# Totoro97/f2-nerf

Hardware: AMD Instinct MI355X
Metric: training ray-samples/s (ngp_fox) (higher is better)
Workload: dtype f16; 1 GPU; ngp_fox wanjinyou.yaml, 8192 rays/batch/GPU, 2^19 x16 table, the first 2188 iterations of training from the fresh-initialised table (fineness 8.7), synthetic random-pose rays, full train step (fwd+bwd+Adam+octree update); rays_per_batch=8192, parallelism=ray-dp1

## Files before the change

### f2-nerf_amd/capi.py

```python
import ctypes
import os

import torch

from . import build

_lib = None
ABI_VERSION = 13


class F2nError(RuntimeError):
    pass


def lib():
    global _lib
    if _lib is None:
        if not os.path.exists(build.LIB):
            raise F2nError("native library %s is missing: run `python -c 'import __graft_entry__ as g; g.build()'` "
                           "(there is no CPU fallback)" % build.LIB)
        _lib = ctypes.CDLL(build.LIB)
        _lib.f2n_build_info.restype = ctypes.c_char_p
        if _lib.f2n_abi_version() != ABI_VERSION:
            raise F2nError("%s reports ABI version %d, this binding is written for %d: rebuild (__graft_entry__.build())"
# ... 454 lines not shown


def draw_ray_batch(n_rays, u01, image_set, height, width, poses, intri, dist_params, images, cam_bounds, cam_indices, ij, rays_o,
                   rays_d, gt_colors, bounds):
    _ck(lib().f2n_draw_ray_batch(_stream(), _i(n_rays), _p(u01, "f32"), _p(image_set, "i32"), _i(int(image_set.numel())), _i(height),
                                 _i(width), _p(poses, "f32"), _p(intri, "f32"), _p(dist_params, "f32"), _p(images, "f32", True),
                                 _p(cam_bounds, "f32"), _p(cam_indices, "i32"), _p(ij, "i32"), _p(rays_o, "f32"), _p(rays_d, "f32"),
                                 _p(gt_colors, "f32", True), _p(bounds, "f32")), "f2n_draw_ray_batch")


def gather_pixels(n, height, width, images, cam_bounds, cam_idx, ij, gt_colors, bounds):
    _ck(lib().f2n_gather_pixels(_stream(), _i(n), _i(height), _i(width), _p(images, "f32", True), _p(cam_bounds, "f32", True),
                                _p(cam_idx, "i32"), _p(ij, "i32"), _p(gt_colors, "f32", True), _p(bounds, "f32", True)),
        "f2n_gather_pixels")


def early_stop(n_rays, pts_se, f0, f0_stride, dt, weights, alphas, mask, kept):
    _ck(lib().f2n_early_stop(_stream(), _i(n_rays), _p(pts_se, "i32"), _p(f0, "f32"), _i(f0_stride), _p(dt, "f32"),
                             _p(weights, "f32"), _p(alphas, "f32"), _p(mask, "i32"), _p(kept, "i32")), "f2n_early_stop")


def compact_samples(n_rays, old_se, new_se, mask, pts, dirs, dt, t, anchors, o_pts, o_dirs, o_dt, o_t, o_anchors):
    _ck(lib().f2n_compact_samples(_stream(), _i(n_rays), _p(old_se, "i32"), _p(new_se, "i32"), _p(mask, "i32"),
                                  _p(pts, "f32"), _p(dirs, "f32"), _p(dt, "f32"), _p(t, "f32"), _p(anchors, "i32"),
                                  _p(o_pts, "f32"), _p(o_dirs, "f32"), _p(o_dt, "f32"), _p(o_t, "f32"),
                                  _p(o_anchors, "i32")), "f2n_compact_samples")


def compact_samples_src(n_rays, old_se, new_se, mask, pts, dirs, dt, t, anchors, o_pts, o_dirs, o_dt, o_t, o_anchors, o_src,
                        o_vol=None, ray_val=None, o_ray_val=None):
    _ck(lib().f2n_compact_samples_src(_stream(), _i(n_rays), _p(old_se, "i32"), _p(new_se, "i32"), _p(mask, "i32"),
                                      _p(pts, "f32"), _p(dirs, "f32"), _p(dt, "f32"), _p(t, "f32"), _p(anchors, "i32"),
                                      _p(o_pts, "f32"), _p(o_dirs, "f32"), _p(o_dt, "f32"), _p(o_t, "f32"),
                                      _p(o_anchors, "i32"), _p(o_src, "i32"), _p(o_vol, "i32", True), _p(ray_val, "i32", True),
                                      _p(o_ray_val, "i32", True)), "f2n_compact_samples_src")


def oct_visible_cams(n_boxes, n_cams, boxes, c2w, bounds, fx, fy, cx, cy, res_h, res_w, pix_i, pix_j, visible):
    _ck(lib().f2n_oct_visible_cams(_stream(), _i(n_boxes), _i(n_cams), _p(boxes, "f32"), _p(c2w, "f32"), _p(bounds, "f32"), _f(fx),
                                   _f(fy), _f(cx), _f(cy), _i(res_h), _i(res_w), _p(pix_i, "f32"), _p(pix_j, "f32"),
                                   _p(visible, "u8")), "f2n_oct_visible_cams")


def march_noise(n, u, fineness, out):
    _ck(lib().f2n_march_noise(_stream(), _i(n), _p(u, "f32"), _f(fineness), _p(out, "f32")), "f2n_march_noise")


def composite_fwd(n_rays, pts_se, feat, dt, t, rgb, bg, colors, disparity, depth, weights, f0_stride=16, out_vars=None):
    _ck(lib().f2n_composite_fwd(_stream(), _i(n_rays), _p(pts_se, "i32"), _p(feat, "f32"), _i(f0_stride), _p(dt, "f32"),
                                _p(t, "f32"), _p(rgb, "f32"), _p(bg, "f32"), _p(colors, "f32"), _p(disparity, "f32"),
                                _p(depth, "f32"), _p(weights, "f32"), _p(out_vars, "f32", True)), "f2n_composite_fwd")


def composite_bwd(n_rays, pts_se, feat, dt, t, rgb, bg, dcolors, ddisp, ddepth, dweights, gs_progress, drgb, dfeat, f0_stride=16,
                  df0_stride=16, var_weights=None, dvars=None):
    _ck(lib().f2n_composite_bwd(_stream(), _i(n_rays), _p(pts_se, "i32"), _p(feat, "f32"), _i(f0_stride), _p(dt, "f32"),
                                _p(t, "f32"), _p(rgb, "f32"), _p(bg, "f32"), _p(dcolors, "f32", True), _p(ddisp, "f32", True),
                                _p(ddepth, "f32", True), _p(dweights, "f32", True), _f(gs_progress), _p(drgb, "f32"),
                                _p(dfeat, "f32"), _i(df0_stride), _p(var_weights, "f32", True), _p(dvars, "f32", True)),
        "f2n_composite_bwd")


def weight_var_fwd(n_rays, weights, pts_se, out):
    _ck(lib().f2n_weight_var_fwd(_stream(), _i(n_rays), _p(weights, "f32"), _p(pts_se, "i32"), _p(out, "f32")),
        "f2n_weight_var_fwd")


# ... 808 lines not shown
```

### f2-nerf_amd/csrc/host/Renderer.cpp

```cpp
#include "Renderer.h"

#include <hip/hip_runtime_api.h>

#include <cstdio>
#include <cstdlib>
#include <mutex>

namespace f2n {

using torch::autograd::AutogradContext;
using torch::autograd::variable_list;

namespace {

struct CompositeFunction : public torch::autograd::Function<CompositeFunction> {
  static variable_list forward(AutogradContext* ctx, Tensor feat, Tensor rgb, Tensor dt, Tensor t, Tensor bg, Tensor se,
                               double gs_progress) {
    ctx->set_materialize_grads(false);
    const int n_rays = se.size(0), m = feat.size(0);
    Tensor colors = torch::empty({n_rays, 3}, DevF32()), disparity = torch::empty({n_rays}, DevF32());
    Tensor depth = torch::empty({n_rays}, DevF32()), weights = torch::empty({m}, DevF32());
    F2N_TIMED_CALL("composite_fwd", f2n_composite_fwd(CurStream(), n_rays, I32P(se), F32P(feat), F2N_MLP_OUT_PAD, F32P(dt), F32P(t), F32P(rgb), F32P(bg),
                               F32P(colors), F32P(disparity), F32P(depth), F32P(weights), nullptr));
    ctx->save_for_backward({feat, rgb, dt, t, bg, se});
// ... 116 lines not shown
  return float(dp_count_host_.data_ptr<int32_t>()[0]) / (float(n_rays) * float(dp_world_));
}

void Renderer::ResolvePendingCount() {
  if (!count_pending_) return;
  count_pending_ = false;
  {
    F2N_HOST_SCOPE("wait.kept");
    kept_wait_ev_->synchronize();
  }
  const int n_kept = n_kept_words_.Read(1);
  last_n_kept_pts_ = n_kept;
  total_kept_pts_ += n_kept;
  DigestKept(pending_count_seq_, n_kept);
  auto* gdp = global_data_pool_;
  if (dp_world_ > 1) {
    if (dp_sum_mirrored_) {
      const float per_ray = float(n_kept_words_.Read(0)) / (float(dp_sum_rays_) * float(dp_world_));
      gdp->meaningful_sampled_pts_per_ray_ = gdp->meaningful_sampled_pts_per_ray_ * 0.9f + per_ray * 0.1f;
      RecordEma(pending_count_seq_ - 1);
    }
    dp_sum_mirrored_ = false;
    return;
  }
  gdp->meaningful_sampled_pts_per_ray_ = gdp->meaningful_sampled_pts_per_ray_ * 0.9f + KeptPerRayForEma(n_kept, pending_count_rays_) * 0.1f;
  RecordEma(pending_count_seq_);
}

RenderFront Renderer::SampleAndFilter(const Tensor& rays_o, const Tensor& rays_d, const Tensor& bounds, const Tensor& emb_idx,
                                      bool async_count) {
  F2N_HOST_SCOPE("step.sample_and_filter");
  auto* gdp = global_data_pool_;
  ResolvePendingCount();
  if (gdp->mode_ == RunningMode::TRAIN) DebugSkew(2);
  auto* field = static_cast<Hash3DAnchored*>(scene_field_.get());
  const bool train = gdp->mode_ == RunningMode::TRAIN;
  const int n_rays = rays_o.size(0);
  spec_start_recorded_ = false;
  spec_start_is_consumed_ = false;
  if (train && async_count && (next_batch_.valid || next2_batch_.valid) && speculative_sampling_ != 0) {
    if (rays_off_main_ && side_shared_ && side_shared_->seq > 0) spec_start_is_consumed_ = true;
    else spec_start_ev_.record();
    spec_start_recorded_ = true;
  }
  auto* ps = static_cast<PersSampler*>(pts_sampler_.get());
  if (train) {
    KeepOnlyPending(rays_o, rays_d, next_batch_.valid ? next_batch_.rays_o : Tensor(), next_batch_.valid ? next_batch_.rays_d : Tensor(),
                    next2_batch_.valid ? next2_batch_.rays_o : Tensor(), next2_batch_.valid ? next2_batch_.rays_d : Tensor());
    const int slot = FindPending(rays_o, rays_d);
    if (slot >= 0) PreSampleFinish(slot);
  } else {
    DropPendingSamples();
  }
  bool wait_for_pack = false;
  int pack_slot = 0;
  auto pack_done = [&]() {
    if (wait_for_pack) presample_done_ev_[pack_slot].block(c10::hip::getCurrentHIPStreamMasqueradingAsCUDA());
    wait_for_pack = false;
  };
  if (train && PresampleMatches(rays_o, rays_d)) {
    sample_result_ = std::move(presampled_);
    if (presample_async_) {
      wait_for_pack = true;
      pack_slot = presample_slot_;
      consumed_side_samples_ = true;
    }
// ... 136 lines not shown
      }
      pack_done();
      if (digest_taps_ && train) {
        DigestTap(TAP_PTS_PRE, sample_result_.pts);
        DigestTap(TAP_DT_PRE, sample_result_.dt);
        DigestTap(TAP_ANCHORS_PRE, sample_result_.anchors.select(1, 0));
      }
      f0_full = field->QueryDensityPreAct(pts_full, anchors_full, true, keep_prepass_outputs_,
                                          keep_prepass_outputs_ && prepass_planes_cache_);
      f0p = F32P(f0_full) + front;
      if (digest_taps_ && train) DigestTap(TAP_EDGE, pts_full.narrow(0, 0, front));
      fr.edge_cache_row = 0;
      fr.sample_cache_row = front;
    } else {
      pack_done();
      if (digest_taps_ && train) {
        DigestTap(TAP_PTS_PRE, sample_result_.pts);
        DigestTap(TAP_DT_PRE, sample_result_.dt);
        DigestTap(TAP_ANCHORS_PRE, sample_result_.anchors.select(1, 0));
      }
      f0_full = field->QueryDensityPreAct(sample_result_.pts, sample_result_.anchors, true, keep_prepass_outputs_,
                                          keep_prepass_outputs_ && prepass_planes_cache_);
      f0p = F32P(f0_full);
    }
    if (digest_taps_ && train) {
      DigestTap(TAP_PTS, sample_result_.pts);
      DigestTap(TAP_DT, sample_result_.dt);
      DigestTap(TAP_ANCHORS, sample_result_.anchors.select(1, 0));
      DigestTap(TAP_F0, f0_full);
      DigestTap(TAP_BG, bg_color);
    }
    Tensor weights = torch::empty({n_all_pts}, DevF32()), alphas = torch::empty({n_all_pts}, DevF32());
    Tensor mask = torch::empty({n_all_pts}, DevI32()), kept = torch::empty({n_rays}, DevI32());
    if (train) ps->EarlyStopAndVote(sample_result_, f0p, weights, alphas, mask, kept);
    else F2N_TIMED_CALL("early_stop", f2n_early_stop(st, n_rays, I32P(sample_result_.pts_idx_bounds), f0p, 1, F32P(sample_result_.dt),
                            F32P(weights), F32P(alphas), I32P(mask), I32P(kept)));
    const bool octree_first = train && async_count;
    auto octree_update_issued = [&]() {
      octree_ready_ev_.record();
      const int nslot = next_batch_.valid ? FindPending(next_batch_.rays_o, next_batch_.rays_d) : -1;
      if (nslot >= 0 && pend_[nslot].s.speculative && !pend_[nslot].s.completed && PreSampleSpecComplete(nslot)) after_octree_update_ = nullptr;
      else if (nslot >= 0 && pend_[nslot].s.completed) after_octree_update_ = nullptr;
      if (after_octree_update_) {
        auto f = std::move(after_octree_update_);
        after_octree_update_ = nullptr;
        f();
      }
    };
    Tensor new_se = torch::empty({n_rays, 2}, DevI32()), total = torch::empty({1}, DevI32());
    n_kept_words_.Ensure(2);
    bool scan_issued = false;
    if (octree_first) {
      PersSampler::ScanArgs sa;
      sa.n = n_rays; sa.counts = I32P(kept); sa.start_end = I32P(new_se); sa.total = I32P(total);
      if (train && dp_world_ > 1 && dp_count_.defined()) {
        sa.mirror = n_kept_words_.Dev(0); sa.also = I32P(dp_count_); sa.n_also = 1;
        dp_sum_mirrored_ = true;
        dp_sum_rays_ = dp_count_rays_;
      } else {
        sa.mirror = n_kept_words_.Dev(1);
      }
      ps->FinishOctUpdate(&sa);
      scan_issued = true;
      octree_update_issued();
    }
    const bool dp_lagged = train && dp_world_ > 1 && octree_first;
    if (scan_issued) {
    } else if (dp_lagged && dp_count_.defined()) {
      F2N_CALL(f2n_segment_scan_ex(st, n_rays, I32P(kept), I32P(new_se), I32P(total), n_kept_words_.Dev(0), I32P(dp_count_), 1));
      dp_sum_mirrored_ = true;
      dp_sum_rays_ = dp_count_rays_;
    } else {
      F2N_CALL(f2n_segment_scan_ex(st, n_rays, I32P(kept), I32P(new_se), I32P(total), n_kept_words_.Dev(1), nullptr, 0));
    }
    kept_wait_ev_ = scan_issued ? &octree_ready_ev_ : &n_kept_ev_;
    if (!scan_issued) n_kept_ev_.record();
    if (digest_taps_ && train) DigestTap(TAP_SURVIVORS, new_se);
    if (dp_lagged) {
      dp_count_ = total;
      dp_count_rays_ = n_rays;
    } else if (train && dp_world_ > 1) {
      dp_count_ = total.clone();
    }
    if (train && !octree_first) ps->FinishOctUpdate();
    if (train && dp_world_ > 1 && !dp_lagged) {
      if (!dp_count_host_.defined()) dp_count_host_ = torch::empty({1}, torch::TensorOptions().dtype(torch::kInt32).pinned_memory(true));
      dp_count_host_.copy_(dp_count_, true);
      dp_count_ev_.record();
    }
    if (train && !octree_first) octree_update_issued();
    if (async_count) {
      n_kept = n_all_pts;
      if (train) {
        count_pending_ = true;
        pending_count_rays_ = n_rays;
        pending_count_seq_ = cur_seq_;
      }
      fr.dyn = true;
      fr.n_kept_dev = total;
    } else {
      kept_wait_ev_->synchronize();
      n_kept = n_kept_words_.Read(1);
      if (train && after_count_readback_) after_count_readback_();
      last_n_kept_pts_ = n_kept;
      if (train) total_kept_pts_ += n_kept;
    }
    const int64_t so = fr.dyn ? 2 * (int64_t) n_edge : 0;
    const int64_t eo = fr.dyn ? 0 : n_kept;
    if (!edges_cached) {
      pts_all = torch::empty({n_kept + 2 * n_edge, 3}, DevF32());
      vol_all = torch::empty({n_kept + 2 * n_edge}, DevI32());
    }
    es.pts = pts_all.slice(0, so, so + n_kept);
    es.dirs = torch::empty({n_kept, 3}, DevF32());
    es.dt = torch::empty({n_kept}, DevF32());
    es.t = torch::empty({n_kept}, DevF32());
    es.anchors = torch::empty({n_kept, 3}, DevI32());
    es.first_oct_dis = sample_result_.first_oct_dis;
    es.pts_idx_bounds = new_se;
    src_rows = torch::empty({std::max(n_kept, 1)}, DevI32());
    const bool want_emb = train && use_app_emb_ && emb_idx.defined();
    Tensor emb_contig;
    if (want_emb) {
      emb_contig = emb_idx.contiguous();
      CheckDev(emb_contig, torch::kInt32, "emb_idx");
      fr.sample_emb_idx = torch::empty({std::max(n_kept, 1)}, DevI32());
    }
    F2N_TIMED_CALL("compact_samples", f2n_compact_samples_src(st, n_rays, I32P(sample_result_.pts_idx_bounds), I32P(new_se), I32P(mask),
                                 F32P(sample_result_.pts), F32P(sample_result_.dirs), F32P(sample_result_.dt),
                                 F32P(sample_result_.t), I32P(sample_result_.anchors), F32P(pts_all) + 3 * so, F32P(es.dirs),
                                 F32P(es.dt), F32P(es.t), I32P(es.anchors), I32P(src_rows), I32P(vol_all) + so,
                                 want_emb ? I32P(emb_contig) : nullptr, want_emb ? I32P(fr.sample_emb_idx) : nullptr));
    if (train) {
      if (!fr.dyn) {
        gdp->meaningful_sampled_pts_per_ray_ = gdp->meaningful_sampled_pts_per_ray_ * 0.9f + KeptPerRayForEma(n_kept, n_rays) * 0.1f;
        RecordEma(cur_seq_);
        DigestKept(cur_seq_, n_kept);
      }
      if (!edges_cached && n_edge > 0) edge_samples_to(F32P(pts_all) + 3 * eo, I32P(vol_all) + eo, 1, nullptr, nullptr);
    }
  }

  fr.n_kept = n_kept;
  fr.n_edge = n_edge;
  fr.side_pool_buffers = pregen;
  fr.emb = train && use_app_emb_ && emb_idx.defined();
  if (!fr.emb) fr.sample_emb_idx = torch::empty({0}, DevI32());
  const bool streaming_train = train && fr.dyn;
  if (streaming_train && consumed_side_samples_) {
    fr.presamples_keepalive = std::move(sample_result_);
    fr.consumed_deferred = true;
    consumed_side_samples_ = false;
  }
  sample_result_ = SampleResultFlex();
  if (consumed_side_samples_) {
    side_shared_->consumed.record();
    consumed_side_samples_ = false;
    side_shared_->seq++;
  }
  if (!streaming_train) octree_ready_ev_.record();
  return fr;
}

RenderResult Renderer::Render(const Tensor& rays_o, const Tensor& rays_d, const Tensor& bounds, const Tensor& emb_idx) {
  auto* gdp = global_data_pool_;
  auto* field = static_cast<Hash3DAnchored*>(scene_field_.get());
  auto* shader = static_cast<SHShader*>(shader_.get());
  const bool train = gdp->mode_ == RunningMode::TRAIN;
  const int n_rays = rays_o.size(0);
  RenderFront fr = SampleAndFilter(rays_o, rays_d, bounds, emb_idx);
  if (fr.empty)
    return {fr.bg_color, torch::zeros({n_rays, 1}, DevF32()), torch::zeros({n_rays}, DevF32()), Tensor(),
            torch::full({n_rays}, 512.f, DevF32()), Tensor(), Tensor()};
  SampleResultFlex& es = fr.es;
  const int n_kept = fr.n_kept, n_edge = fr.n_edge;

  Tensor all_feat = field->AnchoredQueryReuse(fr.pts_all, fr.vol_all, fr.src_rows, n_kept);
  Tensor scene_feat = all_feat.slice(0, 0, n_kept);
  Tensor edge_feat;
  if (train) edge_feat = all_feat.slice(0, n_kept, n_kept + 2 * n_edge).reshape({n_edge, 2, -1});
  Tensor sampled_colors = shader->QueryFromField(scene_feat, es.dirs, fr.emb ? app_emb_ : torch::empty({0}, DevF32()),
                                                 fr.sample_emb_idx, fr.emb ? &app_emb_grad_ : nullptr);
  auto out = CompositeFunction::apply(scene_feat, sampled_colors, es.dt, es.t, fr.bg_color, es.pts_idx_bounds,
                                      (double) gdp->gradient_scaling_progress_);
  return {out[0], es.first_oct_dis, out[1], edge_feat, out[2], out[3], es.pts_idx_bounds, es.dt};
}

RenderResult Renderer::RenderForward(const Tensor& rays_o, const Tensor& rays_d, const Tensor& bounds) {
  auto* gdp = global_data_pool_;
  auto* field = static_cast<Hash3DAnchored*>(scene_field_.get());
  auto* shader = static_cast<SHShader*>(shader_.get());
  TORCH_CHECK(gdp->mode_ != RunningMode::TRAIN, "RenderForward is the inference path");
  if (!FusedPathOk()) return Render(rays_o, rays_d, bounds, Tensor());
  torch::NoGradGuard no_grad;
// ... 55 lines not shown
```

### f2-nerf_amd/csrc/host/Renderer.h

```cpp
#pragma once
#include "Hash3DAnchored.h"
#include "PersSampler.h"

namespace f2n {

class SHShader : public Shader {
 public:
  explicit SHShader(GlobalDataPool* global_data_pool);
  Tensor Query(const Tensor& feats, const Tensor& dirs) override;
  Tensor QueryFromField(const Tensor& field_feats, const Tensor& dirs, const Tensor& app_emb, const Tensor& sample_emb_idx,
                        Tensor* app_emb_grad);
  Tensor SHEncode(const Tensor& dirs);
  std::vector<Tensor> States() override;
  std::vector<ParamGroup> OptimParamGroups() override;
  int LoadStates(const std::vector<Tensor>& states, int idx) override;
  void Reset() override;

  std::unique_ptr<FusedMLP> mlp_;
  int d_hidden_, n_hiddens_, degree_;
  bool fused_ok_ = true;
};

struct RenderResult {
  Tensor colors;
  Tensor first_oct_dis;
  Tensor disparity;
  Tensor edge_feats;
  Tensor depth;
  Tensor weights;
  Tensor idx_start_end;
  Tensor dt;
};

struct RenderFront {
  bool empty = false;
  SampleResultFlex es;
  Tensor pts_all, vol_all;
  Tensor src_rows;
  Tensor bg_color, sample_emb_idx;
  int n_kept = 0, n_edge = 0;
  bool emb = false;
  bool dyn = false;
  Tensor n_kept_dev;
  int64_t edge_cache_row = -1;
  int64_t sample_cache_row = 0;
  bool side_pool_buffers = false;
  SampleResultFlex presamples_keepalive;
  bool consumed_deferred = false;
};

struct GridSpec {
  float lo[3];
  float step;
  int n[3];
};
std::tuple<Tensor, Tensor> MeshFromGrid(const Tensor& grid, float level, const float lo[3], float step);
std::tuple<Tensor, Tensor> MeshFromGridMasked(const Tensor& grid, const Tensor& valid, float level, const float lo[3], float step);
void TsdfIntegrate(const Tensor& S, const Tensor& W, const float lo[3], float step, const Tensor& poses, const Tensor& intri,
                   const Tensor& dist, const Tensor& depth, const Tensor& conf, float trunc);
std::tuple<Tensor, Tensor> TsdfFinalize(const Tensor& S, const Tensor& W, float min_weight);
Tensor GridNormals(const Tensor& grid, const Tensor& pts, const float lo[3], float step);
Tensor MeshComponents(const Tensor& faces, int64_t n_verts, int* rounds = nullptr);
std::tuple<Tensor, Tensor, Tensor> MeshFilterComponents(const Tensor& verts, const Tensor& faces, int min_faces);
std::tuple<Tensor, Tensor, Tensor> MeshSimplify(const Tensor& verts, const Tensor& faces, float cell, const float* lo, double lambda);

struct MeshRaycastAccel {
  float lo[3] = {0.f, 0.f, 0.f}, cell = 1.f;
  int32_t dims[3] = {1, 1, 1};
  Tensor cell_start, cell_faces;
};
float MeshRaycastDefaultCell(const float mn[3], const float mx[3], int64_t n_faces);
MeshRaycastAccel MeshRaycastBuild(const Tensor& verts, const Tensor& faces, float cell, const float* lo);
std::tuple<Tensor, Tensor, Tensor> MeshRaycast(const Tensor& verts, const Tensor& faces, const MeshRaycastAccel* accel, const Tensor& rays_o,
                                               const Tensor& rays_d, const Tensor& bounds);

std::tuple<Tensor, Tensor, Tensor> MeshClosestPoint(const Tensor& verts, const Tensor& faces, const MeshRaycastAccel* accel, const Tensor& points,
                                                    float max_dist);
constexpr uint64_t kMeshSamplePurpose = 0x8CB92BA72F3D8DD7ull;
std::tuple<Tensor, Tensor, Tensor> MeshSampleSurface(const Tensor& verts, const Tensor& faces, int64_t n, uint64_t seed);

struct MeshAtlasResult {
// ... 153 lines not shown
  } ema_ring_[kEmaRing];
  void RecordEma(int64_t seq) {
    if (seq >= 0) ema_ring_[seq % kEmaRing] = {seq, global_data_pool_->meaningful_sampled_pts_per_ray_};
  }
  bool EmaAfter(int64_t seq, float* value) const {
    if (seq < 0 || ema_ring_[seq % kEmaRing].seq != seq) return false;
    *value = ema_ring_[seq % kEmaRing].value;
    return true;
  }
  int64_t pending_count_seq_ = -1;
  static constexpr int kDigestRing = 32768;
  struct StepDigest {
    int64_t seq = -1;
    int iter = 0, n_rays = 0, n_marched = 0, n_kept = -1;
  };
  std::vector<StepDigest> digest_;
  void DigestBegin(int n_rays, int n_marched) {
    if (cur_seq_ < 0) return;
    if (digest_.empty()) digest_.resize(kDigestRing);
    digest_[cur_seq_ % kDigestRing] = {cur_seq_, global_data_pool_->iter_step_, n_rays, n_marched, -1};
  }
  void DigestKept(int64_t seq, int n_kept) {
    if (seq >= 0 && !digest_.empty() && digest_[seq % kDigestRing].seq == seq) digest_[seq % kDigestRing].n_kept = n_kept;
  }
  enum { TAP_PTS, TAP_DT, TAP_ANCHORS, TAP_F0, TAP_SURVIVORS, TAP_BG, TAP_EDGE, TAP_COLORS, TAP_TABLE_GRAD, TAP_SMALL_GRADS, TAP_TABLE,
         TAP_FIELD_MLP, TAP_COLOR_MLP, TAP_APP_EMB, TAP_GRAD_BEFORE, TAP_PTS_ALL_AFTER, TAP_VOL_ALL_AFTER, TAP_FIELD_X, TAP_DFEAT,
         TAP_PTS_PRE, TAP_DT_PRE, TAP_ANCHORS_PRE, TAP_PTS_ALL_PRE, TAP_VOL_ALL_PRE, N_TAPS };
  bool digest_taps_ = false;
  Tensor digest_tap_sums_;
  void DigestTap(int tap, const Tensor& t);
  bool async_count_ = false;
  bool prepass_feat_reuse_ = true;
  bool prepass_planes_cache_ = true;
  bool keep_prepass_outputs_ = false;
  int64_t n_feat_reuse_steps_ = 0;
  bool count_pending_ = false;
  int pending_count_rays_ = 0;
  int64_t total_kept_pts_ = 0, total_all_pts_ = 0;
  TrainOutputs TrainForwardBackward(const Tensor& rays_o, const Tensor& rays_d, const Tensor& bounds, const Tensor& gt_colors,
                                    const Tensor& emb_idx, float var_w, float disp_w, float tv_w, float dist_w = 0.f);

  Tensor QueryDensity(const Tensor& world);
  Tensor DensityGrid(const std::vector<float>& lo, const std::vector<float>& hi, int res);
  std::tuple<Tensor, Tensor> ExtractMesh(const std::vector<float>& lo, const std::vector<float>& hi, int res, float level);
  static GridSpec MakeGridSpec(const std::vector<float>& lo, const std::vector<float>& hi, int res);
  Tensor DensityOfLocated(const Tensor& warped, const Tensor& anchors);
  std::tuple<Tensor, Tensor> QueryRadiance(const Tensor& world, const Tensor& dirs);
  MeshAttrs ExtractMeshAttrs(const std::vector<float>& lo, const std::vector<float>& hi, int res, float level, int min_component_faces,
                             bool normals, bool colors, const std::string& normal_source = "grid", int simplify = 0,
                             const MeshRefineOptions& refine = MeshRefineOptions());
  LevelProjection ProjectToLevel(const Tensor& points, float level, int iters, float max_step, float max_move, float tol,
                                 const Tensor& origins = Tensor());
  std::tuple<Tensor, Tensor> QueryDensityGrad(const Tensor& world);
  Tensor FieldNormals(const Tensor& world);
  void DensityGradSlabs(const Tensor& world, const Tensor& density, const Tensor& grad, const Tensor& normals);
  void DensityGradChunk(const Tensor& world, const Tensor& density, const Tensor& grad, const Tensor& normals);
  GeometryResult RenderGeometry(const Tensor& rays_o, const Tensor& rays_d, const Tensor& bounds, float tau, bool keep_samples);
  int64_t density_slab_points_ = int64_t(1) << 22;

  int LoadStates(const std::vector<Tensor>& states, int idx) override;
  std::vector<Tensor> States() override;
  std::vector<ParamGroup> OptimParamGroups() override;
  void ZeroGrad();
  bool FusedPathOk() const;

  GlobalDataPool* global_data_pool_;
// ... 46 lines not shown
```

### f2-nerf_amd/csrc/host/RendererTrain.cpp

```cpp
#include "Renderer.h"

#include <hip/hip_runtime_api.h>

#include <cstdio>
#include <cstdlib>
#include <mutex>

namespace f2n {

using torch::autograd::AutogradContext;
using torch::autograd::variable_list;

TrainOutputs Renderer::TrainForwardBackward(const Tensor& rays_o, const Tensor& rays_d, const Tensor& bounds,
                                            const Tensor& gt_colors, const Tensor& emb_idx, float var_w, float disp_w, float tv_w,
                                            float dist_w) {
  auto* gdp = global_data_pool_;
  auto* field = static_cast<Hash3DAnchored*>(scene_field_.get());
  auto* shader = static_cast<SHShader*>(shader_.get());
  torch::NoGradGuard no_grad;
  const int n_rays = rays_o.size(0);
  Tensor gt = gt_colors.contiguous();
  CheckDev(gt, torch::kFloat32, "gt_colors");
  TORCH_CHECK(gt.numel() == (int64_t) n_rays * 3, "gt_colors must be [n_rays,3]");
  struct KeepOutputs {
// ... 158 lines not shown
  } else if (reuse) {
    field->grad_clean_ = false;
    F2N_TIMED_CALL("field_bwd", f2n_field_bwd_dyn_rows(st, n, n_dev, 2 * n_edge, field->n_volumes_, I32P(field->prim_pool_),
                           I32P(field->feat_local_idx_), I32P(field->feat_local_size_), F32P(field->bias_pool_),
                           F32P(field->level_scale_), F32P(fr.pts_all), I32P(fr.vol_all), 1, VoidP(field->mlp_->params_h_),
                           x_edge, x_surv, I32P(fr.src_rows), F32P(dfeat), field->mlp_->loss_scale_, F32P(field->mlp_->grad_scaled_),
                           VoidP(field->grad_h_), field->pool_size_ / N_LEVELS, 1));
    F2N_TIMED_CALL("reduce_partials", f2n_reduce_deferred(st));
  } else if (fr.dyn) {
    field->grad_clean_ = false;
    F2N_TIMED_CALL("field_bwd", f2n_field_bwd_dyn(st, n, n_dev, 2 * n_edge, field->n_volumes_, I32P(field->prim_pool_),
                           I32P(field->feat_local_idx_), I32P(field->feat_local_size_), F32P(field->bias_pool_),
                           F32P(field->level_scale_), F32P(fr.pts_all), I32P(fr.vol_all), 1, VoidP(field->mlp_->params_h_),
                           VoidP(field_x), F32P(dfeat), field->mlp_->loss_scale_, F32P(field->mlp_->grad_scaled_),
                           VoidP(field->grad_h_), field->pool_size_ / N_LEVELS, 1));
    F2N_TIMED_CALL("reduce_partials", f2n_reduce_deferred(st));
  } else {
    field->BackwardRaw(fr.pts_all, fr.vol_all, 1, field_x, dfeat);
  }
  if (digest_taps_ && fr.dyn) {
    const int64_t rows = fr.pts_all.size(0);
    Tensor live = torch::arange(rows, DevI32()).lt(fr.n_kept_dev + (int) so).to(torch::kInt32);
    DigestTap(TAP_PTS_ALL_AFTER, fr.pts_all.view(torch::kInt32).sum(1, false, torch::kInt64) * live);
    DigestTap(TAP_VOL_ALL_AFTER, fr.vol_all.to(torch::kInt64) * live);
    Tensor live_n = live.narrow(0, 0, n);
    DigestTap(TAP_FIELD_X, field_x.view(torch::kInt32).sum(1, false, torch::kInt64) * live_n);
    DigestTap(TAP_DFEAT, dfeat.view(torch::kInt32).sum(1, false, torch::kInt64) * live_n);
  }
  if (digest_taps_) {
    DigestTap(TAP_COLORS, colors);
    DigestTap(TAP_TABLE_GRAD, field->grad_h_);
    DigestTap(TAP_SMALL_GRADS, small_grads_flat_);
  }
  if ((fr.side_pool_buffers || fr.consumed_deferred) && side_shared_) {
    side_shared_->consumed.record();
    side_shared_->seq++;
  }
  out.colors = colors;
  out.has_samples = true;
  return out;
}

}
```

### f2-nerf_amd/csrc/host/bindings.cpp

```cpp
#include <torch/extension.h>

#include "DataParallel.h"
#include "ExpRunner.h"

#include <hip/hip_runtime_api.h>

#include <algorithm>

using namespace f2n;

namespace {

Hash3DAnchored* FieldOf(ExpRunner& r) { return static_cast<Hash3DAnchored*>(r.renderer_->scene_field_.get()); }
SHShader* ShaderOf(ExpRunner& r) { return static_cast<SHShader*>(r.renderer_->shader_.get()); }
PersSampler* SamplerOf(ExpRunner& r) { return static_cast<PersSampler*>(r.renderer_->pts_sampler_.get()); }

int g_scatter_producer = 1;

struct InferenceMode {
  GlobalDataPool* gdp;
  RunningMode prev;
  InferenceMode(ExpRunner& r, bool on) : gdp(r.global_data_pool_.get()), prev(gdp->mode_) {
    if (on) gdp->mode_ = RunningMode::VALIDATE;
  }
// ... 691 lines not shown
      .def("step_digest",
           [](ExpRunner& r) {
             r.FinishPending();
             py::list out;
             auto& dg = r.renderer_->digest_;
             Tensor sums = r.digest_table_sums_.defined() ? r.digest_table_sums_.cpu() : Tensor();
             std::vector<Renderer::StepDigest> rows;
             for (auto& d : dg) if (d.seq >= 0) rows.push_back(d);
             std::sort(rows.begin(), rows.end(), [](const Renderer::StepDigest& a, const Renderer::StepDigest& b) { return a.seq < b.seq; });
             for (auto& d : rows) {
               py::list row;
               row.append(d.seq); row.append(d.iter); row.append(d.n_rays); row.append(d.n_marched); row.append(d.n_kept);
               if (sums.defined()) row.append(sums.data_ptr<int64_t>()[d.seq % Renderer::kDigestRing]);
               out.append(row);
             }
             return out;
           })
      .def_readwrite("iter_step", &ExpRunner::iter_step_)
      .def_readwrite("check_nan", &ExpRunner::check_nan_)
      .def_readwrite("async_counts", &ExpRunner::async_counts_)
      .def_property("speculative_sampling",
                    [](ExpRunner& r) { return r.renderer_->speculative_sampling_; },
                    [](ExpRunner& r, int mode) { r.renderer_->speculative_sampling_ = mode; })
      .def_property("tail_repair",
                    [](ExpRunner& r) { return static_cast<PersSampler*>(r.renderer_->pts_sampler_.get())->tail_repair_; },
                    [](ExpRunner& r, bool on) { static_cast<PersSampler*>(r.renderer_->pts_sampler_.get())->tail_repair_ = on; })
      .def_readwrite("fused_tail", &ExpRunner::fused_tail_)
      .def_property("prepass_feat_reuse",
                    [](ExpRunner& r) { return r.renderer_->prepass_feat_reuse_; },
                    [](ExpRunner& r, bool on) { r.renderer_->prepass_feat_reuse_ = on; })
      .def_property("prepass_planes_cache",
                    [](ExpRunner& r) { return r.renderer_->prepass_planes_cache_; },
                    [](ExpRunner& r, bool on) { r.renderer_->prepass_planes_cache_ = on; })
      .def_property_readonly("prepass_reuse_steps", [](ExpRunner& r) { return r.renderer_->n_feat_reuse_steps_; })
      .def_property("scatter_producer",
                    [](ExpRunner&) { return g_scatter_producer; },
                    [](ExpRunner&, int variant) {
                      if (f2n_set_scatter_producer(variant) != F2N_OK) throw std::invalid_argument("scatter_producer: 0 or 1");
                      g_scatter_producer = variant;
                    })
      .def_readwrite("spec_start_without_event", &ExpRunner::spec_start_without_event_)
      .def_readwrite("draws_off_main", &ExpRunner::draws_off_main_)
      .def_readwrite("exact_flag_order", &ExpRunner::exact_flag_order_)
      .def_property("march_block_waves",
                    [](ExpRunner& r) { return static_cast<PersSampler*>(r.renderer_->pts_sampler_.get())->march_block_waves_; },
                    [](ExpRunner& r, int n) { static_cast<PersSampler*>(r.renderer_->pts_sampler_.get())->march_block_waves_ = std::min(16, std::max(1, n)); })
      .def_property("march_blocks",
                    [](ExpRunner& r) { return static_cast<PersSampler*>(r.renderer_->pts_sampler_.get())->march_blocks_; },
                    [](ExpRunner& r, int n) { static_cast<PersSampler*>(r.renderer_->pts_sampler_.get())->march_blocks_ = std::max(0, n); })
      .def_property("speculation_depth",
                    [](ExpRunner& r) { return r.renderer_->spec_depth_; },
                    [](ExpRunner& r, int d) { r.FinishPending(); r.renderer_->DropPendingSamples(); r.renderer_->spec_depth_ = std::max(1, std::min(3, d)); })
      .def("speculation_counters",
           [](ExpRunner& r) {
             r.FinishPending();
             py::dict d;
             d["speculative"] = r.renderer_->n_speculative_;
             d["fallback"] = r.renderer_->n_spec_fallback_;
             d["dropped"] = r.renderer_->n_spec_dropped_;
             auto& o = *SamplerOf(r)->pers_octree_;
             d["rays_repaired"] = o.n_repaired_.defined() ? o.n_repaired_.item<int>() : 0;
             d["stat_updates"] = o.epoch_;
             return d;
           })
      .def("counters",
           [](ExpRunner& r) {
// ... 16 lines not shown
```

### f2-nerf_amd/csrc/render.hip

```cpp
#include "rows_dev.h"


__global__ __launch_bounds__(256) void early_stop_kernel(int n_rays, const int32_t* __restrict__ se, const float* __restrict__ f0,
                                                         int f0_stride, const float* __restrict__ dt, float* __restrict__ weights,
                                                         float* __restrict__ alphas, int32_t* __restrict__ mask,
                                                         int32_t* __restrict__ kept) {
  F2N_RAISE_PRIO();
  const int c = threadIdx.x & 15;
  const int ray = blockIdx.x * F2N_ROW_RAYS_PER_BLOCK + (threadIdx.x >> 4);
  if (ray >= n_rays) return;
  const int s = se[2 * ray], e = se[2 * ray + 1];
  float acc = 0.f;
  int cnt = 0;
  float n_f0 = 0.f, n_dt = 0.f;
  if (s < e) {
    const int i = min(s + c, e - 1);
    n_f0 = f0[(size_t) i * f0_stride];
    n_dt = dt[i];
  }
  for (int base = s; base < e; base += 16) {
    const int i = base + c;
    const bool in = i < e;
    const float c_f0 = n_f0, c_dt = n_dt;
    if (base + 16 < e) {
// ... 15 lines not shown
    }
    cnt += m;
  }
#pragma unroll
  for (int off = 8; off >= 1; off >>= 1) cnt += __shfl_xor(cnt, off, 16);
  if (c == 0) kept[ray] = cnt;
}

__global__ __launch_bounds__(256) void compact_kernel(int n_rays, const int32_t* __restrict__ old_se,
                                                      const int32_t* __restrict__ new_se, const int32_t* __restrict__ mask,
                                                      const float* __restrict__ pts, const float* __restrict__ dirs,
                                                      const float* __restrict__ dt, const float* __restrict__ t,
                                                      const int32_t* __restrict__ anchors, float* __restrict__ o_pts,
                                                      float* __restrict__ o_dirs, float* __restrict__ o_dt, float* __restrict__ o_t,
                                                      int32_t* __restrict__ o_anchors, int32_t* __restrict__ o_src,
                                                      int32_t* __restrict__ o_vol, const int32_t* __restrict__ ray_val,
                                                      int32_t* __restrict__ o_ray_val) {
  const int lane = threadIdx.x & 63;
  const int ray = blockIdx.x * (blockDim.x / 64) + (threadIdx.x >> 6);
  if (ray >= n_rays) return;
  const int s = old_se[2 * ray], e = old_se[2 * ray + 1];
  int dst = new_se[2 * ray];
  const int rv = o_ray_val != nullptr ? ray_val[ray] : 0;
  for (int base = s; base < e; base += 64) {
    const int i = base + lane;
    const bool keep = i < e && mask[i] != 0;
    const unsigned long long bal = __ballot(keep);
    if (keep) {
      const int k = dst + __popcll(bal & ((1ull << lane) - 1ull));
#pragma unroll
      for (int c = 0; c < 3; c++) {
        o_pts[3 * (size_t) k + c] = pts[3 * (size_t) i + c];
        o_dirs[3 * (size_t) k + c] = dirs[3 * (size_t) i + c];
        o_anchors[3 * (size_t) k + c] = anchors[3 * (size_t) i + c];
      }
      o_dt[k] = dt[i];
      o_t[k] = t[i];
      if (o_src != nullptr) o_src[k] = i;
      if (o_vol != nullptr) o_vol[k] = anchors[3 * (size_t) i];
      if (o_ray_val != nullptr) o_ray_val[k] = rv;
    }
    dst += __popcll(bal);
  }
}

__device__ __forceinline__ void f2n_wv_stats(const float* __restrict__ w, int n, int c, float& mean, float& wsum) {
  float m = 0.f, ws = 1e-6f;
  for (int base = 0; base < n; base += 16) {
    const int i = base + c;
    const float wi = i < n ? w[i] : 0.f;
    m = f2n_row_last(f2n_row_seq_scan(wi * ((float) i / 16.f), m, c));
    ws = f2n_row_last(f2n_row_seq_scan(wi, ws, c));
  }
  mean = m / ws;
  wsum = ws;
}

__global__ __launch_bounds__(256) void composite_fwd_kernel(int n_rays, const int32_t* __restrict__ se, const float* __restrict__ f0,
                                                            int f0_stride, const float* __restrict__ dt, const float* __restrict__ t,
                                                            const float* __restrict__ rgb, const float* __restrict__ bg,
                                                            float* __restrict__ colors, float* __restrict__ disparity,
                                                            float* __restrict__ depth, float* __restrict__ weights,
                                                            float* __restrict__ out_vars) {
  F2N_RAISE_PRIO();
  const int c = threadIdx.x & 15;
  const int ray = blockIdx.x * F2N_ROW_RAYS_PER_BLOCK + (threadIdx.x >> 4);
  if (ray >= n_rays) return;
// ... 904 lines not shown
```

Baseline: 713.4 million ray-samples/s.

## Move octree vote update onto tail stream and skip unused anchor compaction

When training with async counting on a single device and no maintenance step is due, the octree node vote update now runs on a separate tail stream, ordered after an early-stop event. The main stream can then continue with the scan and compaction instead of waiting for the votes. The votes are joined back at the next sample step or after backward. Separately, compact_samples no longer writes per-sample anchors when the dynamic training path does not need them, which saves memory traffic. The cost is extra event synchronisation, longer-lived weight and alpha tensors, and a risk of ordering bugs between the octree update and the next presample.

```diff
diff --git a/f2-nerf_amd/capi.py b/f2-nerf_amd/capi.py
--- a/f2-nerf_amd/capi.py
+++ b/f2-nerf_amd/capi.py
@@ -510,7 +510,7 @@
     _ck(lib().f2n_compact_samples_src(_stream(), _i(n_rays), _p(old_se, "i32"), _p(new_se, "i32"), _p(mask, "i32"),
                                       _p(pts, "f32"), _p(dirs, "f32"), _p(dt, "f32"), _p(t, "f32"), _p(anchors, "i32"),
                                       _p(o_pts, "f32"), _p(o_dirs, "f32"), _p(o_dt, "f32"), _p(o_t, "f32"),
-                                      _p(o_anchors, "i32"), _p(o_src, "i32"), _p(o_vol, "i32", True), _p(ray_val, "i32", True),
+                                      _p(o_anchors, "i32", True), _p(o_src, "i32"), _p(o_vol, "i32", True), _p(ray_val, "i32", True),
                                       _p(o_ray_val, "i32", True)), "f2n_compact_samples_src")
 
 
diff --git a/f2-nerf_amd/csrc/host/Renderer.cpp b/f2-nerf_amd/csrc/host/Renderer.cpp
--- a/f2-nerf_amd/csrc/host/Renderer.cpp
+++ b/f2-nerf_amd/csrc/host/Renderer.cpp
@@ -172,6 +172,7 @@
   F2N_HOST_SCOPE("step.sample_and_filter");
   auto* gdp = global_data_pool_;
   ResolvePendingCount();
+  JoinTailVotes();
   if (gdp->mode_ == RunningMode::TRAIN) DebugSkew(2);
   auto* field = static_cast<Hash3DAnchored*>(scene_field_.get());
   const bool train = gdp->mode_ == RunningMode::TRAIN;
@@ -374,12 +375,22 @@
     }
     Tensor weights = torch::empty({n_all_pts}, DevF32()), alphas = torch::empty({n_all_pts}, DevF32());
     Tensor mask = torch::empty({n_all_pts}, DevI32()), kept = torch::empty({n_rays}, DevI32());
-    if (train) ps->EarlyStopAndVote(sample_result_, f0p, weights, alphas, mask, kept);
+    const bool votes_off = train && async_count && votes_off_main_ != 0 && dp_world_ == 1 && !ps->occupancy_sync_hook_ &&
+                           !ps->MaintenanceDue(0) && !digest_taps_ && (votes_off_main_ == 1 || !two_deep);
+    Tensor new_se = torch::empty({n_rays, 2}, DevI32()), total = torch::empty({1}, DevI32());
+    n_kept_words_.Ensure(2);
+    if (votes_off) {
+      ps->VoteBuffer();
+      F2N_TIMED_CALL("early_stop", f2n_early_stop(st, n_rays, I32P(sample_result_.pts_idx_bounds), f0p, 1, F32P(sample_result_.dt),
+                              F32P(weights), F32P(alphas), I32P(mask), I32P(kept)));
+      F2N_CALL(f2n_segment_scan_ex(st, n_rays, I32P(kept), I32P(new_se), I32P(total), n_kept_words_.Dev(1), nullptr, 0));
+    } else if (train) ps->EarlyStopAndVote(sample_result_, f0p, weights, alphas, mask, kept);
     else F2N_TIMED_CALL("early_stop", f2n_early_stop(st, n_rays, I32P(sample_result_.pts_idx_bounds), f0p, 1, F32P(sample_result_.dt),
                             F32P(weights), F32P(alphas), I32P(mask), I32P(kept)));
     const bool octree_first = train && async_count;
-    auto octree_update_issued = [&]() {
-      octree_ready_ev_.record();
+    auto octree_update_issued = [&](c10::hip::HIPStreamMasqueradingAsCUDA* on = nullptr) {
+      if (on != nullptr) octree_ready_ev_.record(*on);
+      else octree_ready_ev_.record();
       const int nslot = next_batch_.valid ? FindPending(next_batch_.rays_o, next_batch_.rays_d) : -1;
       if (nslot >= 0 && pend_[nslot].s.speculative && !pend_[nslot].s.completed && PreSampleSpecComplete(nslot)) after_octree_update_ = nullptr;
       else if (nslot >= 0 && pend_[nslot].s.completed) after_octree_update_ = nullptr;
@@ -389,10 +400,25 @@
         f();
       }
     };
-    Tensor new_se = torch::empty({n_rays, 2}, DevI32()), total = torch::empty({1}, DevI32());
-    n_kept_words_.Ensure(2);
     bool scan_issued = false;
-    if (octree_first) {
+    if (votes_off) {
+      early_stop_ev_.record();
+      auto* tail = TailStream();
+      early_stop_ev_.block(*tail);
+      TORCH_CHECK(!ps->occupancy_sync_hook_ && !ps->MaintenanceDue(0), "votes off the main queue: not on a step with an exchange or octree maintenance");
+      fr.votes_weights = weights;
+      fr.votes_alphas = alphas;
+      fr.votes_deferred = true;
+      fr.votes_join = std::shared_ptr<void>(nullptr, [this](void*) { try { JoinTailVotes(); } catch (...) {} });
+      tail_votes_pending_ = true;
+      {
+        c10::hip::HIPStreamGuardMasqueradingAsCUDA guard(*tail);
+        ps->UpdateOctNodes(sample_result_, weights, alphas);
+      }
+      n_votes_off_main_steps_++;
+      scan_issued = true;
+      octree_update_issued(tail);
+    } else if (octree_first) {
       PersSampler::ScanArgs sa;
       sa.n = n_rays; sa.counts = I32P(kept); sa.start_end = I32P(new_se); sa.total = I32P(total);
       if (train && dp_world_ > 1 && dp_count_.defined()) {
@@ -415,7 +441,7 @@
     } else {
       F2N_CALL(f2n_segment_scan_ex(st, n_rays, I32P(kept), I32P(new_se), I32P(total), n_kept_words_.Dev(1), nullptr, 0));
     }
-    kept_wait_ev_ = scan_issued ? &octree_ready_ev_ : &n_kept_ev_;
+    kept_wait_ev_ = votes_off ? &early_stop_ev_ : scan_issued ? &octree_ready_ev_ : &n_kept_ev_;
     if (!scan_issued) n_kept_ev_.record();
     if (digest_taps_ && train) DigestTap(TAP_SURVIVORS, new_se);
     if (dp_lagged) {
@@ -457,7 +483,8 @@
     es.dirs = torch::empty({n_kept, 3}, DevF32());
     es.dt = torch::empty({n_kept}, DevF32());
     es.t = torch::empty({n_kept}, DevF32());
-    es.anchors = torch::empty({n_kept, 3}, DevI32());
+    const bool want_anchors = !(train && fr.dyn);
+    if (want_anchors) es.anchors = torch::empty({n_kept, 3}, DevI32());
     es.first_oct_dis = sample_result_.first_oct_dis;
     es.pts_idx_bounds = new_se;
     src_rows = torch::empty({std::max(n_kept, 1)}, DevI32());
@@ -471,7 +498,7 @@
     F2N_TIMED_CALL("compact_samples", f2n_compact_samples_src(st, n_rays, I32P(sample_result_.pts_idx_bounds), I32P(new_se), I32P(mask),
                                  F32P(sample_result_.pts), F32P(sample_result_.dirs), F32P(sample_result_.dt),
                                  F32P(sample_result_.t), I32P(sample_result_.anchors), F32P(pts_all) + 3 * so, F32P(es.dirs),
-                                 F32P(es.dt), F32P(es.t), I32P(es.anchors), I32P(src_rows), I32P(vol_all) + so,
+                                 F32P(es.dt), F32P(es.t), want_anchors ? I32P(es.anchors) : nullptr, I32P(src_rows), I32P(vol_all) + so,
                                  want_emb ? I32P(emb_contig) : nullptr, want_emb ? I32P(fr.sample_emb_idx) : nullptr));
     if (train) {
       if (!fr.dyn) {
@@ -493,6 +520,8 @@
     fr.presamples_keepalive = std::move(sample_result_);
     fr.consumed_deferred = true;
     consumed_side_samples_ = false;
+  } else if (fr.votes_deferred) {
+    fr.presamples_keepalive = std::move(sample_result_);
   }
   sample_result_ = SampleResultFlex();
   if (consumed_side_samples_) {
@@ -502,6 +531,12 @@
   }
   if (!streaming_train) octree_ready_ev_.record();
   return fr;
+}
+
+void Renderer::JoinTailVotes() {
+  if (!tail_votes_pending_) return;
+  octree_ready_ev_.block(c10::hip::getCurrentHIPStreamMasqueradingAsCUDA());
+  tail_votes_pending_ = false;
 }
 
 RenderResult Renderer::Render(const Tensor& rays_o, const Tensor& rays_d, const Tensor& bounds, const Tensor& emb_idx) {
diff --git a/f2-nerf_amd/csrc/host/Renderer.h b/f2-nerf_amd/csrc/host/Renderer.h
--- a/f2-nerf_amd/csrc/host/Renderer.h
+++ b/f2-nerf_amd/csrc/host/Renderer.h
@@ -47,6 +47,9 @@
   bool side_pool_buffers = false;
   SampleResultFlex presamples_keepalive;
   bool consumed_deferred = false;
+  Tensor votes_weights, votes_alphas;
+  bool votes_deferred = false;
+  std::shared_ptr<void> votes_join;
 };
 
 struct GridSpec {
@@ -266,6 +269,11 @@
   bool async_count_ = false;
   bool prepass_feat_reuse_ = true;
   bool prepass_planes_cache_ = true;
+  int votes_off_main_ = 2;
+  int64_t n_votes_off_main_steps_ = 0;
+  at::cuda::CUDAEvent early_stop_ev_;
+  bool tail_votes_pending_ = false;
+  void JoinTailVotes();
   bool keep_prepass_outputs_ = false;
   int64_t n_feat_reuse_steps_ = 0;
   bool count_pending_ = false;
diff --git a/f2-nerf_amd/csrc/host/RendererTrain.cpp b/f2-nerf_amd/csrc/host/RendererTrain.cpp
--- a/f2-nerf_amd/csrc/host/RendererTrain.cpp
+++ b/f2-nerf_amd/csrc/host/RendererTrain.cpp
@@ -214,6 +214,7 @@
     DigestTap(TAP_TABLE_GRAD, field->grad_h_);
     DigestTap(TAP_SMALL_GRADS, small_grads_flat_);
   }
+  if (fr.votes_deferred) JoinTailVotes();
   if ((fr.side_pool_buffers || fr.consumed_deferred) && side_shared_) {
     side_shared_->consumed.record();
     side_shared_->seq++;
diff --git a/f2-nerf_amd/csrc/host/bindings.cpp b/f2-nerf_amd/csrc/host/bindings.cpp
--- a/f2-nerf_amd/csrc/host/bindings.cpp
+++ b/f2-nerf_amd/csrc/host/bindings.cpp
@@ -747,6 +747,13 @@
       .def_property("prepass_planes_cache",
                     [](ExpRunner& r) { return r.renderer_->prepass_planes_cache_; },
                     [](ExpRunner& r, bool on) { r.renderer_->prepass_planes_cache_ = on; })
+      .def_property("votes_off_main",
+                    [](ExpRunner& r) { return r.renderer_->votes_off_main_; },
+                    [](ExpRunner& r, int mode) {
+                      if (mode < 0 || mode > 2) throw std::invalid_argument("votes_off_main: 0, 1 or 2");
+                      r.renderer_->votes_off_main_ = mode;
+                    })
+      .def_property_readonly("votes_off_main_steps", [](ExpRunner& r) { return r.renderer_->n_votes_off_main_steps_; })
       .def_property_readonly("prepass_reuse_steps", [](ExpRunner& r) { return r.renderer_->n_feat_reuse_steps_; })
       .def_property("scatter_producer",
                     [](ExpRunner&) { return g_scatter_producer; },
diff --git a/f2-nerf_amd/csrc/render.hip b/f2-nerf_amd/csrc/render.hip
--- a/f2-nerf_amd/csrc/render.hip
+++ b/f2-nerf_amd/csrc/render.hip
@@ -71,7 +71,10 @@
       for (int c = 0; c < 3; c++) {
         o_pts[3 * (size_t) k + c] = pts[3 * (size_t) i + c];
         o_dirs[3 * (size_t) k + c] = dirs[3 * (size_t) i + c];
-        o_anchors[3 * (size_t) k + c] = anchors[3 * (size_t) i + c];
+      }
+      if (o_anchors != nullptr) {
+#pragma unroll
+        for (int c = 0; c < 3; c++) o_anchors[3 * (size_t) k + c] = anchors[3 * (size_t) i + c];
       }
       o_dt[k] = dt[i];
       o_t[k] = t[i];
```

Measured after the change: 731.3 million ray-samples/s, median of 6. +2.5%, better.
